# pucgenie/JAADec

Measured on AMD Instinct MI355X. Metric: AAC frames/sec (batched) at 1/2/4/8 MI355X; PCM ±1 LSB vs Java ref, higher is better.
Workload: dtype f32; 1 GPU; C2: 65536 AAC-LC 48 kHz stereo frames (256 streams x 256), ONLY_LONG windows; frames_per_gpu=65536, frames_per_job=65536, streams_per_job=256, parallelism=stream-sharded x1 (no collectives), pcm=int16 big-endian, samples_per_frame=1024, lc_kernel=long-window instantiation

## Files before the change

jaadec_amd/csrc/jaad_lc.hip:

```cpp
#include <hip/hip_runtime.h>

#include <algorithm>

#include "jaad_lc.h"

namespace jaad {

__device__ __forceinline__ int lane_id()
{
    int v;
    asm volatile("v_mbcnt_lo_u32_b32 %0, -1, 0\n\tv_mbcnt_hi_u32_b32 %0, -1, %0" : "=v"(v));
    __builtin_assume(v >= 0 && v < 64);
    return v;
}

__device__ __forceinline__ int lane_pos(int u)
{
    return (u >> 3) | ((int)(__builtin_bitreverse32((uint32_t)u) >> 29) << 3);
}

__device__ __forceinline__ void wave_sync()
{
    __builtin_amdgcn_fence(__ATOMIC_RELEASE, "wavefront");
    __builtin_amdgcn_wave_barrier();
// ... 863 lines not shown
        else if (j == 2) { n = 2 * k + 64; v = re[s]; }
        else { n = 319 - 2 * k; v = re[s]; }
    }
}

__device__ __forceinline__ void ola_short(float* Tb, const LdsTables& T, int u, const FrameCtx& fc,
                                          const float (&re)[8], const float (&im)[8], float (&ov)[16],
                                          float (&out)[16])
{
    const int w = u >> 3, b = u & 7;
    const float* SWc = T.win_short[fc.shape];
    const float* SWr = T.win_short[w == 0 ? fc.shape_prev : fc.shape];
    float nv[16];
#pragma unroll
    for (int phase = 0; phase < 2; phase++) {
#pragma unroll
        for (int s = 0; s < 8; s++) {
#pragma unroll
            for (int j = 0; j < 4; j++) {
                int n;
                float v;
                short_slot(b, s, j, re, im, n, v);
                if ((n < 128) != (phase == 1)) continue;
                if (phase == 0) Tb[128 * w + (n - 128)] = v * SWc[255 - n];
                else Tb[128 * w + n] = v * SWr[n];
            }
        }
        wave_sync();
        const int uu = lane_id();
#pragma unroll
        for (int o = 0; o < 16; o++) {
            const int P = long_pos(uu, o);
            const int mo = (P - 448) >> 7, io = (P - 448) & 127;
            const int mq = (P + 576) >> 7, iq = (P + 576) & 127;
            if (phase == 0) {
                out[o] = (P >= 448 + 128) ? ov[o] + Tb[128 * (mo - 1) + io] : ov[o];
                nv[o] = (mq <= 8) ? Tb[128 * (mq - 1) + iq] : 0.0f;
            } else {
                if (P >= 448) out[o] = out[o] + Tb[128 * mo + io];
                if (mq <= 7) nv[o] = nv[o] + Tb[128 * mq + iq];
            }
        }
        wave_sync();
    }
#pragma unroll
    for (int o = 0; o < 16; o++) ov[o] = nv[o];
}

__device__ __forceinline__ void ola_short2(float* TL, float* TR, const LdsTables& T, int u, const FrameCtx& fL,
                                           const FrameCtx& fR, const float (&reL)[8], const float (&imL)[8],
                                           const float (&reR)[8], const float (&imR)[8], float (&ovL)[16],
                                           float (&ovR)[16], float (&outL)[16], float (&outR)[16])
{
    const int w = u >> 3, b = u & 7;
    const float* SWcL = T.win_short[fL.shape];
    const float* SWrL = T.win_short[w == 0 ? fL.shape_prev : fL.shape];
    const float* SWcR = T.win_short[fR.shape];
    const float* SWrR = T.win_short[w == 0 ? fR.shape_prev : fR.shape];
    float nvL[16], nvR[16];
#pragma unroll
    for (int phase = 0; phase < 2; phase++) {
#pragma unroll
        for (int s = 0; s < 8; s++) {
#pragma unroll
            for (int j = 0; j < 4; j++) {
                int n;
                float vl, vr;
                short_slot(b, s, j, reL, imL, n, vl);
                short_slot(b, s, j, reR, imR, n, vr);
                if ((n < 128) != (phase == 1)) continue;
                if (phase == 0) {
                    TL[128 * w + (n - 128)] = vl * SWcL[255 - n];
                    TR[128 * w + (n - 128)] = vr * SWcR[255 - n];
                } else {
                    TL[128 * w + n] = vl * SWrL[n];
                    TR[128 * w + n] = vr * SWrR[n];
                }
            }
        }
        wave_sync();
        const int uu = lane_id();
#pragma unroll
        for (int o = 0; o < 16; o++) {
            const int P = long_pos(uu, o);
            const int mo = (P - 448) >> 7, io = (P - 448) & 127;
            const int mq = (P + 576) >> 7, iq = (P + 576) & 127;
            if (phase == 0) {
                outL[o] = (P >= 448 + 128) ? ovL[o] + TL[128 * (mo - 1) + io] : ovL[o];
                outR[o] = (P >= 448 + 128) ? ovR[o] + TR[128 * (mo - 1) + io] : ovR[o];
                nvL[o] = (mq <= 8) ? TL[128 * (mq - 1) + iq] : 0.0f;
                nvR[o] = (mq <= 8) ? TR[128 * (mq - 1) + iq] : 0.0f;
            } else {
                if (P >= 448) {
                    outL[o] = outL[o] + TL[128 * mo + io];
                    outR[o] = outR[o] + TR[128 * mo + io];
                }
                if (mq <= 7) {
                    nvL[o] = nvL[o] + TL[128 * mq + iq];
                    nvR[o] = nvR[o] + TR[128 * mq + iq];
                }
            }
        }
        wave_sync();
    }
#pragma unroll
    for (int o = 0; o < 16; o++) {
        ovL[o] = nvL[o];
        ovR[o] = nvR[o];
    }
}

__device__ void tns_spec(float* buf, float* scratch, const LdsTables& T, const GlobalTables& G, int u,
                         const Ics& info, const jaad_tns* tp)
{
    const bool is_short = info.seq == JAAD_EIGHT_SHORT_SEQUENCE;
    const int nswb = is_short ? T.nswb_s : T.nswb_l;
    const int16_t* offs = is_short ? G.swb_s : G.swb_l;
    const int tns_max = is_short ? T.tns_max_s : T.tns_max_l;
    const int nf = tp->n_filters;
    if (u < nf && u < 8) {
        const jaad_tns_filter& F = tp->filt[u];
        int top = nswb, bottom = nswb;
        for (int f = 0; f <= u; f++) {
            const jaad_tns_filter& G = tp->filt[f];
            if (G.window != F.window) continue;
            top = bottom;
            bottom = top - G.length;
            if (bottom < 0) bottom = 0;
        }
        const int order = F.order > 20 ? 20 : F.order;
        float* a = scratch + 24 * u;
        float bb[21];
        const float* tab = G.tns_coef[2 * ((F.flags >> 2) & 1) + ((F.flags >> 1) & 1)];
        a[0] = 1.0f;
        for (int m = 1; m <= order; m++) {
            float tm = -tab[F.coef[m - 1] & 15];
            for (int i = 1; i < m; i++) bb[i] = a[i] + tm * a[m - i];
            for (int i = 1; i < m; i++) a[i] = bb[i];
            a[m] = tm;
        }
        int s = bottom < tns_max ? bottom : tns_max;
        if (s > info.max_sfb) s = info.max_sfb;
        int e = top < tns_max ? top : tns_max;
        if (e > info.max_sfb) e = info.max_sfb;
        int start = offs[s], end = offs[e];
        int size = end - start;
        if (order > 0 && size > 0) {
            int inc = 1;
            if (F.flags & 1) {
                inc = -1;
                start = end - 1;
            }
            const int base = (is_short ? 128 * (F.window & 7) : 0) + start;
            for (int n = 0; n < size; n++) {
                float y = buf[eo_idx(base + n * inc)];
                for (int j = 0; j < order; j++) {
                    float st = (n - 1 - j >= 0) ? buf[eo_idx(base + (n - 1 - j) * inc)] : 0.0f;
                    y -= st * a[j + 1];
                }
                buf[eo_idx(base + n * inc)] = y;
            }
        }
    }
    wave_sync();
}

__device__ __forceinline__ void store_spec(float* buf, int u, const float (&x)[16])
{
#pragma unroll
    for (int h = 0; h < 2; h++) {
        const int p = 8 * u + 512 * h;
        *reinterpret_cast<float4*>(&buf[eo_idx(p)]) = make_float4(x[8 * h], x[8 * h + 2], x[8 * h + 4], x[8 * h + 6]);
        *reinterpret_cast<float4*>(&buf[eo_idx(p + 1)]) =
            make_float4(x[8 * h + 1], x[8 * h + 3], x[8 * h + 5], x[8 * h + 7]);
    }
}
__device__ __forceinline__ void load_spec(const float* buf, int u, float (&x)[16])
{
#pragma unroll
    for (int h = 0; h < 2; h++) {
        const int p = 8 * u + 512 * h;
        float4 e = *reinterpret_cast<const float4*>(&buf[eo_idx(p)]);
        float4 o = *reinterpret_cast<const float4*>(&buf[eo_idx(p + 1)]);
        x[8 * h + 0] = e.x; x[8 * h + 2] = e.y; x[8 * h + 4] = e.z; x[8 * h + 6] = e.w;
        x[8 * h + 1] = o.x; x[8 * h + 3] = o.y; x[8 * h + 5] = o.z; x[8 * h + 7] = o.w;
    }
}

typedef int v4i __attribute__((ext_vector_type(4)));
typedef unsigned v4u __attribute__((ext_vector_type(4)));

__device__ __forceinline__ uint32_t round_pk16(float a, float b)
{
    int ia, ib;
    uint32_t w;
    asm("v_cvt_rpi_i32_f32 %0, %1" : "=v"(ia) : "v"(a));
    asm("v_cvt_rpi_i32_f32 %0, %1" : "=v"(ib) : "v"(b));
    asm("v_cvt_pk_i16_i32 %0, %1, %2" : "=v"(w) : "v"(ia), "v"(ib));
    return w;
}

__device__ __forceinline__ uint32_t round_pk16_lsb1(float a, float b)
{
    f2 x = f2{a, b};
    if constexpr (!kScaledOut) x = x * f2{kPcmUnit, kPcmUnit};
    uint32_t w;
    asm("v_cvt_pknorm_i16_f32 %0, %1, %2" : "=v"(w) : "v"(x.x), "v"(x.y));
    return w;
}

__device__ __forceinline__ void vmem_drain() { __builtin_amdgcn_s_waitcnt(0x0F70); }

__device__ __forceinline__ __amdgpu_buffer_rsrc_t frame_rsrc(void* base, int bytes)
{
    return __builtin_amdgcn_make_buffer_rsrc(base, (short)0, bytes, 0x00020000);
}
__device__ __forceinline__ void store16(v4u v, __amdgpu_buffer_rsrc_t r, int off, bool nt)
{
    if (nt) __builtin_amdgcn_raw_buffer_store_b128(v, r, off, 0, 2);
    else __builtin_amdgcn_raw_buffer_store_b128(v, r, off, 0, 0);
}

constexpr int kRspFloats = kWaveBuf;
template <bool kTns>
struct alignas(16) WaveLds {
    float buf[kWaveBuf];
    float rsp[kRspFloats];
};
template <>
struct alignas(16) WaveLds<true> {
    float buf[kWaveBuf];
    float rsp[kRspFloats];
    float tns[192];
};
#ifndef JAAD_LC_WAVES
#define JAAD_LC_WAVES 12
#endif
template <bool kTns>
constexpr int waves_per_wg()
{
    return kTns ? 8 : JAAD_LC_WAVES;
}

struct alignas(16) BandRec {
    float gl, ms, gr, is;
};
constexpr int kNoBand = 127;
constexpr float kZeroBandGain = -0.0f;

__device__ __forceinline__ int band_short(const LdsTables& T, const Ics& ic, int p)
{
    const int w = p >> 7;
    const int sfb = T.quad2band_s[(p & 127) >> 2];
    const int g = w - __builtin_popcount(ic.grouping & ((1u << w) - 1u));
    return sfb < ic.max_sfb ? g * ic.max_sfb + sfb : kNoBand;
}

__device__ void pns_fill(float* buf, const uint32_t* raw, const LdsTables& T, const GlobalTables& G, int u,
                         const Ics& info)
{
    if (u == 0) {
        const uint8_t* sfr = reinterpret_cast<const uint8_t*>(raw);
        const uint8_t* cbr = sfr + 128;
        const bool is_short = info.seq == JAAD_EIGHT_SHORT_SEQUENCE;
        const int16_t* offs = is_short ? G.swb_s : G.swb_l;
        int glen[8], ng = 1;
        glen[0] = 1;
        if (is_short)
            for (int i = 0; i < 7; i++) {
                if (info.grouping & (1u << i)) glen[ng - 1]++;
                else glen[ng++] = 1;
            }
        uint32_t rs = info.pns;
        const int maxSFB = info.max_sfb;
        for (int g = 0, idx = 0, groupOff = 0; g < ng; g++) {
            for (int sfb = 0; sfb < maxSFB; sfb++, idx++) {
                if (cbr[idx] != JAAD_NOISE_HCB) continue;
                int off = groupOff + offs[sfb];
                const int width = offs[sfb + 1] - offs[sfb];
                const float sfv = -T.sf_gain[sfr[idx]];
                for (int w = 0; w < glen[g]; w++, off += 128) {
                    float energy = 0.0f;
                    for (int k = 0; k < width; k++) {
                        rs = 1664525u * rs + 1013904223u;
                        const float v = (float)(int32_t)rs;
                        buf[eo_idx(off + k)] = v;
                        energy += v * v;
                    }
                    const float scale = (float)((double)sfv / sqrt((double)energy));
                    for (int k = 0; k < width; k++) buf[eo_idx(off + k)] *= scale;
                }
            }
            groupOff += glen[g] << 7;
        }
    }
    wave_sync();
}

struct Prefetch {
    v4i q[2][2];
    uint32_t sf2[2], cb2[2];
    uint32_t side;
};

__device__ __forceinline__ void prefetch(const KernelArgs& A, int f, bool stereo, int u, Prefetch& pf, int skip = 0)
{
    const int nch = stereo ? 2 : 1;
#pragma unroll
    for (int c = 0; c < 2; c++) {
        if (c == 1 && !stereo) break;
        const size_t cf = (size_t)f * A.cf_stride + c;
        const v4i* q = reinterpret_cast<const v4i*>(A.q + cf * 1024);
        pf.q[c][0] = __builtin_nontemporal_load(q + u);
        pf.q[c][1] = __builtin_nontemporal_load(q + 64 + u);
        pf.sf2[c] = reinterpret_cast<const uint16_t*>(A.sf + cf * 128)[u];
        pf.cb2[c] = reinterpret_cast<const uint16_t*>(A.cb + cf * 128)[u];
    }
    const uint32_t* side = u < 8 ? reinterpret_cast<const uint32_t*>(A.ics + (size_t)f * A.cf_stride) + (u < 4 * nch ? u : 0)
                                 : (A.ms_used ? reinterpret_cast<const uint32_t*>(A.ms_used + (size_t)f * 2 * A.ms_stride) + (u & 3)
                                              : reinterpret_cast<const uint32_t*>(A.ics));
    if (A.skips && u >= 62) side = A.skips + 2 * skip + (u == 62);
    pf.side = *side;
}

__device__ __forceinline__ void iq_channel(const LdsTables& T, const float* iq_global, const v4i (&q)[2],
                                           const float (&g)[4], float (&x)[16])
{
    float v[16];
    typedef unsigned short us2 __attribute__((ext_vector_type(2)));
    static_assert(kIqHead == 1024, "escape mask assumes a 2048-entry head");
    uint32_t t[8];
#pragma unroll
    for (int d = 0; d < 8; d++) {
        const uint32_t w = reinterpret_cast<const uint32_t*>(&q[d >> 2])[d & 3];
        t[d] = __builtin_bit_cast(uint32_t, __builtin_bit_cast(us2, w) + (us2){kIqHead, kIqHead});
    }
    const bool esc = ((t[0] | t[1] | t[2] | t[3] | t[4] | t[5] | t[6] | t[7]) & 0xF800F800u) != 0u;
#pragma unroll
    for (int e = 0; e < 16; e++) {
        const uint32_t idx = (e & 1) ? (t[e >> 1] >> 16) : (t[e >> 1] & 0xFFFFu);
        v[e] = T.iq_signed[idx];
    }
    __builtin_amdgcn_sched_group_barrier(0x0002, 8, 0);
#pragma unroll
    for (int e = 0; e < 16; e++) {
        __builtin_amdgcn_sched_group_barrier(0x0002, 1, 0);
        __builtin_amdgcn_sched_group_barrier(0x0100, 1, 0);
    }
    __builtin_amdgcn_sched_group_barrier(0x0002, 64, 0);
#pragma unroll
    for (int e = 0; e < 16; e++) {
        const float gn = g[e >> 2];
        x[e] = v[e] * gn;
    }
    if (__builtin_expect(__ballot(esc) != 0, 0)) {
#pragma unroll
        for (int e = 0; e < 16; e++) {
            const int qq = reinterpret_cast<const int16_t*>(&q[e >> 3])[e & 7];
            const int qc = qq < -kIqHead ? -kIqHead : (qq > kIqHead - 1 ? kIqHead - 1 : qq);
            const int aq = qq < 0 ? -qq : qq;
            const float gn = g[e >> 2];
            const float m = iq_global[aq > 8190 ? 8190 : aq] * gn;
            const bool big = (qq > kIqHead - 1 || qq < -kIqHead) && gn != 0.0f;
            x[e] = big ? (qq > 0 ? m : -m) : T.iq_signed[qc + kIqHead] * gn;
        }
    }
}

struct IqPending {
    float v[16];
    bool esc;
};
__device__ __forceinline__ void iq_issue(const LdsTables& T, const v4i (&q)[2], IqPending& P)
{
    typedef unsigned short us2 __attribute__((ext_vector_type(2)));
    uint32_t t[8];
#pragma unroll
    for (int d = 0; d < 8; d++) {
        const uint32_t w = reinterpret_cast<const uint32_t*>(&q[d >> 2])[d & 3];
        t[d] = __builtin_bit_cast(uint32_t, __builtin_bit_cast(us2, w) + (us2){kIqHead, kIqHead});
    }
    P.esc = ((t[0] | t[1] | t[2] | t[3] | t[4] | t[5] | t[6] | t[7]) & 0xF800F800u) != 0u;
#pragma unroll
    for (int e = 0; e < 16; e++) {
        const uint32_t idx = (e & 1) ? (t[e >> 1] >> 16) : (t[e >> 1] & 0xFFFFu);
        P.v[e] = T.iq_signed[idx];
    }
}
__device__ __forceinline__ void iq_finish(const LdsTables& T, const float* iq_global, const v4i (&q)[2],
                                          const IqPending& P, const float (&g)[4], float (&x)[16])
{
#pragma unroll
    for (int e = 0; e < 16; e++) x[e] = P.v[e] * g[e >> 2];
    if (__builtin_expect(__ballot(P.esc) != 0, 0)) {
#pragma unroll
        for (int e = 0; e < 16; e++) {
            const int qq = reinterpret_cast<const int16_t*>(&q[e >> 3])[e & 7];
            const int qc = qq < -kIqHead ? -kIqHead : (qq > kIqHead - 1 ? kIqHead - 1 : qq);
            const int aq = qq < 0 ? -qq : qq;
            const float gn = g[e >> 2];
            const float m = iq_global[aq > 8190 ? 8190 : aq] * gn;
            const bool big = (qq > kIqHead - 1 || qq < -kIqHead) && gn != 0.0f;
            x[e] = big ? (qq > 0 ? m : -m) : T.iq_signed[qc + kIqHead] * gn;
        }
    }
}

__device__ __forceinline__ void couple_after_tns(const KernelArgs& A, float* buf, int f, int ch, int u)
{
    const uint32_t t0 = A.cce_off[f], t1 = A.cce_off[f + 1];
    bool any = false;
    float x[16];
    for (uint32_t t = t0; t < t1; t++) {
        const uint32_t meta = A.cce_meta[t];
        if (!(meta >> 24) || (int)((meta >> 16) & 0xFF) - (int)A.ch0 != ch) continue;
        if (!any) load_spec(buf, u, x);
        any = true;
        const float4* sp = reinterpret_cast<const float4*>(A.cce_spec + (size_t)t * 1024);
#pragma unroll
        for (int h = 0; h < 2; h++) {
            const float4 a = sp[(512 * h + 8 * u) / 4], c = sp[(512 * h + 8 * u) / 4 + 1];
            const float v[8] = {a.x, a.y, a.z, a.w, c.x, c.y, c.z, c.w};
#pragma unroll
            for (int i = 0; i < 8; i++) x[8 * h + i] += v[i];
        }
    }
    if (any) {
        store_spec(buf, u, x);
        wave_sync();
    }
}

template <bool kTnsSpec, bool kCoupleAfter = false, bool F = false>
__device__ __forceinline__ void synth_channel(const KernelArgs& A, const LdsTables& T, WaveLds<kTnsSpec>& W, float* buf,
                                              const Ics& ic, size_t cf, float (&ov)[16], float (&out)[16], int f = 0,
                                              int ch = 0)
{
    const int u = lane_id();
    if constexpr (kTnsSpec)
        if (A.tns_mode == JAAD_TNS_SPEC && (ic.flags & JAAD_ICS_TNS) && A.tns) tns_spec(buf, W.tns, T, *A.gtab, u, ic, A.tns + cf);
    if constexpr (kCoupleAfter) couple_after_tns(A, buf, f, ch, u);
    const FrameCtx fc{ic.seq, ic.shape, ic.shape_prev};
    if (fc.seq == JAAD_EIGHT_SHORT_SEQUENCE) {
        float re[8], im[8];
        imdct_short_pk<F>(buf, T, u, re, im);
        ola_short(buf, T, u, fc, re, im, ov, out);
    } else {
        float* const bufs[1] = {buf};
        f2 cx[1][8];
        imdct_long_pk<1, F>(bufs, T, u, cx);
        ola_long_pk<F>(T, fc, cx[0], ov, out);
    }
    wave_sync();
}

#ifdef JAAD_STAMPS
#define STAMP(k)                                                  \
    do {                                                          \
        uint64_t t_;                                              \
        asm volatile("s_memtime %0\n\ts_waitcnt lgkmcnt(0)" : "=s"(t_)::"memory"); \
        st_acc[k] += (uint32_t)(t_ - st_prev);                    \
        st_prev = t_;                                             \
    } while (0)
#elif defined(JAAD_MARKS)
#define STAMP(k) asm volatile(";PHASE " #k)
#else
#define STAMP(k) \
    do {         \
    } while (0)
#endif

#ifdef JAAD_BOUNDS
#define JAAD_BOUND(ci, f, cond, what, a, b)                                                                 \
    do {                                                                                                   \
        if (!(cond)) {                                                                                     \
            if (lane_id() == 0)                                                                            \
                printf("JAAD_BOUNDS lc_decode_kernel: chunk %u frame %d: %s %u vs %u\n", (unsigned)(ci), (int)(f), \
                       what, (unsigned)(a), (unsigned)(b));                                                \
            return;                                                                                        \
        }                                                                                                  \
    } while (0)
#else
#define JAAD_BOUND(ci, f, cond, what, a, b) \
    do {                                    \
    } while (0)
#endif

template <int kMode, int kOut, bool kStereo>
__global__ __launch_bounds__(64 * waves_per_wg<kMode == 1 || kMode == 3>()) void lc_decode_kernel(KernelArgs A)
{
    constexpr bool kTnsSpec = kMode == 1 || kMode == 3;
    [[maybe_unused]] constexpr bool kCouple = kMode == 2 || kMode == 3;
    constexpr bool kFast = kMode == 4 || kMode == 6;
    [[maybe_unused]] constexpr bool kShortPair = kMode == 5 || kMode == 6;
    constexpr int kW = waves_per_wg<kTnsSpec>();
    constexpr int kThreads = 64 * kW;
    struct Lds {
        LdsTables T;
        WaveLds<kTnsSpec> W[kW];
        uint32_t rem[kW];
    };
    __shared__ Lds S;
    LdsTables& T = S.T;

    {
        const uint4* src = reinterpret_cast<const uint4*>(A.tables);
        uint4* dst = reinterpret_cast<uint4*>(&T);
        for (int i = threadIdx.x; i < (int)(sizeof(LdsTables) / 16); i += kThreads) dst[i] = src[i];
        if (threadIdx.x < kW) S.rem[threadIdx.x] = 0u;
    }
    __syncthreads();
#ifdef JAAD_WAVETIME
    const uint64_t wt0 = __builtin_amdgcn_s_memrealtime();
    uint32_t wt_frames = 0;
#endif

    constexpr bool big_endian = !(kOut & JAAD_PCM_LITTLE_ENDIAN);
    constexpr bool planar = kOut == (int)kOutPlanarF32;
    constexpr bool out_f32 = (kOut & JAAD_PCM_FLOAT32) != 0 && !planar;
    [[maybe_unused]] constexpr bool out_i16 = !planar && !out_f32;
    const int wave = __builtin_amdgcn_readfirstlane(threadIdx.x >> 6);
    constexpr bool stereo = kStereo;
    constexpr int nch = stereo ? 2 : 1;
    WaveLds<kTnsSpec>& W = S.W[wave];
    BandRec* rec = reinterpret_cast<BandRec*>(W.buf);

    const int nswb_l = __builtin_amdgcn_readfirstlane(T.nswb_l), nswb_s = __builtin_amdgcn_readfirstlane(T.nswb_s);
    uint32_t q2b_long = 0;
    {
        const int u = lane_id();
#pragma unroll
        for (int qd = 0; qd < 4; qd++) {
            const uint32_t b = T.quad2band_l[(512 * (qd >> 1) + 8 * u + 4 * (qd & 1)) >> 2];
            q2b_long |= (b > kNoBand ? kNoBand : b) << (8 * qd);
        }
    }

#ifdef JAAD_STAMPS
    uint32_t st_acc[16] = {};
    uint64_t st_prev;
    asm volatile("s_memtime %0\n\ts_waitcnt lgkmcnt(0)" : "=s"(st_prev)::"memory");
#endif
    for (uint32_t ci = blockIdx.x * kW + wave; ci < A.n_chunks; ci += gridDim.x * kW) {
        const ChunkDesc cd = A.chunks[ci];
        const int nfr = cd.info & 0xffff;
        const bool prefix = (cd.info & kChunkPrefix) != 0;
        const int my_n = nfr + (prefix ? 1 : 0);
        const int f_first = (int)cd.frame0;
        JAAD_BOUND(ci, -1, cd.slot < A.n_slots, "chunk slot", cd.slot, A.n_slots);
        JAAD_BOUND(ci, f_first, my_n == 0 || (cd.frame0 >= A.frame_lo && cd.frame0 + (uint32_t)my_n <= A.frame_hi),
                   "chunk frames", cd.frame0 + (uint32_t)my_n, A.frame_hi);
        JAAD_BOUND(ci, f_first, !A.skips || cd.skip < A.n_skip_pairs, "chunk skip entry", cd.skip, A.n_skip_pairs);
        if (cd.slot >= A.n_slots || (my_n && (cd.frame0 < A.frame_lo || cd.frame0 >= A.frame_hi))) continue;

        float ovL[16], ovR[16];
        {
            const int u = lane_id();
            if (cd.info & kChunkLoadState) {
                const float* st = A.state_in + (size_t)cd.slot * 2048;
#pragma unroll
                for (int o = 0; o < 16; o++) {
                    ovL[o] = st[long_pos(u, o)];
                    ovR[o] = st[1024 + long_pos(u, o)];
                    if constexpr (kFast && kScaledOut) {
                        ovL[o] *= kPcmUnit;
                        ovR[o] *= kPcmUnit;
                    }
                }
            } else {
#pragma unroll
                for (int o = 0; o < 16; o++) ovL[o] = ovR[o] = 0.0f;
            }
        }
        int skip = (int)cd.skip;
        int fr_next = f_first;
        Prefetch pf;
        if (my_n > 0) prefetch(A, fr_next, stereo, lane_id(), pf, skip);
        vmem_drain();

        for (int it = 0; it < my_n; it++) {
#if !defined(JAAD_ABL_NOPRIO)
#ifndef JAAD_PRIO_EVERY
#define JAAD_PRIO_EVERY 1
#endif
            if ((it % JAAD_PRIO_EVERY) == 0) {
                const uint32_t rem = (uint32_t)(my_n - it);
                int p = 0;
                if constexpr (kFast) {
                    __hip_atomic_store(&S.rem[wave], rem, __ATOMIC_RELAXED, __HIP_MEMORY_SCOPE_WORKGROUP);
                    uint32_t mates[kW / 4 - 1];
#pragma unroll
                    for (int m = 1; m < kW / 4; m++)
                        mates[m - 1] = __hip_atomic_load(&S.rem[(wave + 4 * m) % kW], __ATOMIC_RELAXED, __HIP_MEMORY_SCOPE_WORKGROUP);
                    static_assert(kW <= 16, "the key keeps the wave in 4 bits");
                    const uint32_t key = (rem << 4) | (uint32_t)wave;
#pragma unroll
                    for (int m = 1; m < kW / 4; m++) {
                        const uint32_t mate = (uint32_t)((wave + 4 * m) % kW);
                        p += key > ((__builtin_amdgcn_readfirstlane(mates[m - 1]) << 4) | mate) ? 1 : 0;
                    }
                } else {
                    volatile uint32_t* R = S.rem;
                    R[wave] = rem;
#pragma unroll
                    for (int m = 1; m < kW / 4; m++) {
                        const int mate = (wave + 4 * m) % kW;
                        const uint32_t r = __builtin_amdgcn_readfirstlane(R[mate]);
                        p += (rem > r || (rem == r && wave > mate)) ? 1 : 0;
                    }
                }
                if (p >= 2) __builtin_amdgcn_s_setprio(3);
                else if (p == 1) __builtin_amdgcn_s_setprio(2);
                else __builtin_amdgcn_s_setprio(1);
            }
#endif
            STAMP(5);
#ifdef JAAD_WAVETIME
            wt_frames++;
#endif
            const int u = lane_id();
            const bool emit = it >= (prefix ? 1 : 0);
            const int f = fr_next;
            const size_t cf0 = (size_t)f * A.cf_stride;
            const Prefetch cur = pf;
            fr_next = f + 1;
            if (A.skips && fr_next == __builtin_amdgcn_readlane(cur.side, 63)) {
                fr_next += __builtin_amdgcn_readlane(cur.side, 62);
                skip++;
            }
            JAAD_BOUND(ci, f, (uint32_t)f >= A.frame_lo && (uint32_t)f < A.frame_hi, "frame rows / pcm", f, A.frame_hi);
            JAAD_BOUND(ci, f, it + 1 >= my_n || ((uint32_t)fr_next >= A.frame_lo && (uint32_t)fr_next < A.frame_hi),
                       "prefetched frame", fr_next, A.frame_hi);
            JAAD_BOUND(ci, f, !A.skips || (uint32_t)skip < A.n_skip_pairs, "skip entry", skip, A.n_skip_pairs);
            if constexpr (kCouple) {
                JAAD_BOUND(ci, f, A.cce_off[f] <= A.cce_off[f + 1] && A.cce_off[f + 1] <= A.n_cce_terms, "coupling terms",
                           A.cce_off[f + 1], A.n_cce_terms);
            }

#if defined(JAAD_NO_IQ_EARLY)
            constexpr bool kIqEarly = false;
#else
            constexpr bool kIqEarly = kFast;
#endif
            [[maybe_unused]] IqPending iqL, iqR;
            if constexpr (kIqEarly) {
                iq_issue(T, cur.q[0], iqL);
                if (stereo) iq_issue(T, cur.q[1], iqR);
            }
            const Ics iL = ics_from_lanes(cur.side, 0, nswb_l, nswb_s);
            STAMP(6);
            const Ics iR = stereo ? ics_from_lanes(cur.side, 4, nswb_l, nswb_s) : iL;
            const bool ms_on = stereo && (iL.flags & JAAD_ICS_COMMON_WINDOW) && (iL.flags & JAAD_ICS_MS_PRESENT);
            const bool is_on = stereo && (iR.flags & JAAD_ICS_HAS_IS);
            const bool same_bands = !stereo || (iL.seq == iR.seq && iL.max_sfb == iR.max_sfb && iL.grouping == iR.grouping);
            uint64_t m0 = 0, m1 = 0;
            if (ms_on && A.ms_used) {
                m0 = (uint64_t)(uint32_t)__builtin_amdgcn_readlane(cur.side, 8) |
                     ((uint64_t)(uint32_t)__builtin_amdgcn_readlane(cur.side, 9) << 32);
                m1 = (uint64_t)(uint32_t)__builtin_amdgcn_readlane(cur.side, 10) |
                     ((uint64_t)(uint32_t)__builtin_amdgcn_readlane(cur.side, 11) << 32);
            }

            STAMP(0);
            {
                const uint32_t sfL2 = cur.sf2[0], cbL2 = cur.cb2[0];
                const uint32_t sfR2 = stereo ? cur.sf2[1] : 0u, cbR2 = stereo ? cur.cb2[1] : 0u;
                const uint64_t mw = u < 32 ? m0 : m1;
                const uint32_t msb = (uint32_t)(mw >> ((2 * u) & 63)) & 3u;
                BandRec br[2];
#pragma unroll
                for (int e = 0; e < 2; e++) {
                    const int b = 2 * u + e;
                    const uint32_t sfL = (sfL2 >> (8 * e)) & 255u, cbL = (cbL2 >> (8 * e)) & 255u;
                    const uint32_t sfR = (sfR2 >> (8 * e)) & 255u, cbR = (cbR2 >> (8 * e)) & 255u;
                    const bool inL = b < iL.nbands, inR = b < iR.nbands;
                    const bool msbit = (msb >> e) & 1u;
                    const float gvL = T.sf_gain[sfL];
                    br[e].gl = (inL && cbL != JAAD_ZERO_HCB && cbL < JAAD_NOISE_HCB) ? gvL : kZeroBandGain;
                    br[e].ms = (ms_on && inL && msbit && cbL < JAAD_NOISE_HCB && cbR < JAAD_NOISE_HCB) ? 1.0f : 0.0f;
                    float gr = 0.0f, is = 0.0f;
                    if (stereo) {
                        const float gvR = T.sf_gain[sfR];
                        gr = (inR && cbR != JAAD_ZERO_HCB && cbR < JAAD_NOISE_HCB) ? gvR : kZeroBandGain;
                        if (is_on && inR && (cbR == JAAD_INTENSITY_HCB || cbR == JAAD_INTENSITY_HCB2)) {
                            float cs = cbR == JAAD_INTENSITY_HCB ? 1.0f : -1.0f;
                            if ((iL.flags & JAAD_ICS_MS_PRESENT) && msbit) cs = -cs;
                            is = cs * gvR;
                        }
                    }
                    br[e].gr = gr;
                    br[e].is = is;
                }
                wave_sync();
                reinterpret_cast<float4*>(rec)[2 * u] = make_float4(br[0].gl, br[0].ms, br[0].gr, br[0].is);
                reinterpret_cast<float4*>(rec)[2 * u + 1] = make_float4(br[1].gl, br[1].ms, br[1].gr, br[1].is);
            }
            wave_sync();

            STAMP(1);
            float gL[4], gR[4], msq[4], isq[4];
            uint32_t q2b = q2b_long;
            asm volatile("" : "+v"(q2b));
            if (iL.seq != JAAD_EIGHT_SHORT_SEQUENCE && same_bands) {
#pragma unroll
                for (int qd = 0; qd < 4; qd++) {
                    const float4 r = reinterpret_cast<const float4*>(rec)[(q2b >> (8 * qd)) & 255u];
                    gL[qd] = r.x;
                    msq[qd] = r.y;
                    gR[qd] = r.z;
                    isq[qd] = r.w;
                }
            } else {
#pragma unroll
                for (int qd = 0; qd < 4; qd++) {
                    const int p = 512 * (qd >> 1) + 8 * u + 4 * (qd & 1);
                    const int bl = iL.seq == JAAD_EIGHT_SHORT_SEQUENCE ? band_short(T, iL, p) : (int)((q2b >> (8 * qd)) & 255u);
                    const float4 r = reinterpret_cast<const float4*>(rec)[bl];
                    gL[qd] = r.x;
                    msq[qd] = r.y;
                    if (same_bands) {
                        gR[qd] = r.z;
                        isq[qd] = r.w;
                    } else {
                        const int br = iR.seq == JAAD_EIGHT_SHORT_SEQUENCE ? band_short(T, iR, p) : (int)((q2b >> (8 * qd)) & 255u);
                        const float2 rr = reinterpret_cast<const float2*>(rec)[2 * br + 1];
                        gR[qd] = rr.x;
                        isq[qd] = rr.y;
                    }
                }
            }
            float xL[16], xR[16];
            STAMP(14);
            if constexpr (kIqEarly) {
                iq_finish(T, A.iq_table, cur.q[0], iqL, gL, xL);
                STAMP(13);
                if (stereo) iq_finish(T, A.iq_table, cur.q[1], iqR, gR, xR);
            } else {
                iq_channel(T, A.iq_table, cur.q[0], gL, xL);
                STAMP(13);
                if (stereo) iq_channel(T, A.iq_table, cur.q[1], gR, xR);
            }
            STAMP(12);
#ifdef JAAD_ABL_NOPREF
            if (it == 0)
#endif
            prefetch(A, it + 1 < my_n ? fr_next : f, stereo, u, pf, skip);

            if ((iL.flags | (stereo ? iR.flags : 0)) & JAAD_ICS_HAS_PNS) {
                uint32_t* rcopy = reinterpret_cast<uint32_t*>(W.rsp);
                wave_sync();
                {
                    uint16_t* r16 = reinterpret_cast<uint16_t*>(rcopy);
                    r16[u] = (uint16_t)cur.sf2[0];
                    r16[64 + u] = (uint16_t)cur.cb2[0];
                    if (stereo) {
                        r16[128 + u] = (uint16_t)cur.sf2[1];
                        r16[192 + u] = (uint16_t)cur.cb2[1];
                    }
                }
                if (iL.flags & JAAD_ICS_HAS_PNS) {
                    wave_sync();
                    store_spec(W.buf, u, xL);
                    wave_sync();
                    pns_fill(W.buf, rcopy, T, *A.gtab, u, iL);
                    load_spec(W.buf, u, xL);
                }
                if (stereo && (iR.flags & JAAD_ICS_HAS_PNS)) {
                    wave_sync();
                    store_spec(W.buf, u, xR);
                    wave_sync();
                    pns_fill(W.buf, rcopy + 64, T, *A.gtab, u, iR);
                    load_spec(W.buf, u, xR);
                }
            }
            STAMP(2);
            if (ms_on) {
#pragma unroll
                for (int qd = 0; qd < 4; qd++) {
                    if (msq[qd] != 0.0f) {
#pragma unroll
                        for (int i = 0; i < 4; i++) {
                            const int e = 8 * (qd >> 1) + 4 * (qd & 1) + i;
                            const float l = xL[e], r = xR[e];
                            xL[e] = l + r;
                            xR[e] = l - r;
                        }
                    }
                }
            }
            if (is_on) {
#pragma unroll
                for (int qd = 0; qd < 4; qd++) {
                    if (isq[qd] != 0.0f) {
#pragma unroll
                        for (int i = 0; i < 4; i++) {
                            const int e = 8 * (qd >> 1) + 4 * (qd & 1) + i;
                            xR[e] = xL[e] * isq[qd];
                        }
                    }
                }
            }

            if constexpr (kCouple) {
                const uint32_t t0 = A.cce_off[f], t1 = A.cce_off[f + 1];
                for (uint32_t t = t0; t < t1; t++) {
                    if (kMode == 3 && (A.cce_meta[t] >> 24)) break;
                    const int ch = (int)((A.cce_meta[t] >> 16) & 0xFF) - (int)A.ch0;
                    if (ch < 0 || ch >= nch) continue;
                    const float4* sp = reinterpret_cast<const float4*>(A.cce_spec + (size_t)t * 1024);
                    float v[16];
#pragma unroll
                    for (int h = 0; h < 2; h++) {
                        const float4 a = sp[(512 * h + 8 * u) / 4], c = sp[(512 * h + 8 * u) / 4 + 1];
                        v[8 * h + 0] = a.x;
                        v[8 * h + 1] = a.y;
                        v[8 * h + 2] = a.z;
                        v[8 * h + 3] = a.w;
                        v[8 * h + 4] = c.x;
                        v[8 * h + 5] = c.y;
                        v[8 * h + 6] = c.z;
                        v[8 * h + 7] = c.w;
                    }
                    if (ch == 0) {
#pragma unroll
                        for (int e = 0; e < 16; e++) xL[e] += v[e];
                    } else {
                        if constexpr (stereo) {
#pragma unroll
                            for (int e = 0; e < 16; e++) xR[e] += v[e];
                        }
                    }
                }
            }

            STAMP(3);
            wave_sync();
            store_spec(W.buf, u, xL);
            if (stereo) store_spec(W.rsp, u, xR);
            wave_sync();
            STAMP(4);
            float outL[16], outR[16];
            if (stereo && iL.seq != JAAD_EIGHT_SHORT_SEQUENCE && iR.seq != JAAD_EIGHT_SHORT_SEQUENCE) {
                if constexpr (kTnsSpec) {
                    if (A.tns_mode == JAAD_TNS_SPEC && A.tns) {
                        if (iL.flags & JAAD_ICS_TNS) tns_spec(W.buf, W.tns, T, *A.gtab, u, iL, A.tns + cf0);
                        if (iR.flags & JAAD_ICS_TNS) tns_spec(W.rsp, W.tns, T, *A.gtab, u, iR, A.tns + cf0 + 1);
                    }
                }
                if constexpr (kMode == 3) {
                    couple_after_tns(A, W.buf, f, 0, u);
                    couple_after_tns(A, W.rsp, f, 1, u);
                }
                float* const bufs[2] = {W.buf, W.rsp};
                f2 cx[2][8];
                imdct_long_pk<2, kFast>(bufs, T, lane_id(), cx);
                ola_long_pk<kFast>(T, FrameCtx{iL.seq, iL.shape, iL.shape_prev}, cx[0], ovL, outL);
                ola_long_pk<kFast>(T, FrameCtx{iR.seq, iR.shape, iR.shape_prev}, cx[1], ovR, outR);
                wave_sync();
            } else if (kShortPair && stereo && iL.seq == JAAD_EIGHT_SHORT_SEQUENCE && iR.seq == JAAD_EIGHT_SHORT_SEQUENCE) {
                float reL[8], imL[8], reR[8], imR[8];
                imdct_short_pk2<kFast>(W.buf, W.rsp, T, lane_id(), reL, imL, reR, imR);
                ola_short2(W.buf, W.rsp, T, lane_id(), FrameCtx{iL.seq, iL.shape, iL.shape_prev},
                           FrameCtx{iR.seq, iR.shape, iR.shape_prev}, reL, imL, reR, imR, ovL, ovR, outL, outR);
                wave_sync();
            } else {
                synth_channel<kTnsSpec, kMode == 3, kFast>(A, T, W, W.buf, iL, cf0, ovL, outL, f, 0);
                if (stereo) synth_channel<kTnsSpec, kMode == 3, kFast>(A, T, W, W.rsp, iR, cf0 + 1, ovR, outR, f, 1);
            }
            STAMP(8);
            vmem_drain();
            STAMP(9);
            {
                const int u2 = lane_id();
                const int drop = emit ? 0 : 4096;
                if constexpr (planar) {
#pragma unroll
                    for (int o = 0; o < 16; o++) {
                        W.buf[long_pos(u2, o)] = kFast && kScaledOut ? outL[o] * kPcmScale : outL[o];
                        if (stereo) W.rsp[long_pos(u2, o)] = kFast && kScaledOut ? outR[o] * kPcmScale : outR[o];
                    }
                    wave_sync();
#pragma unroll
                    for (int c = 0; c < nch; c++) {
                        const __amdgpu_buffer_rsrc_t dst = frame_rsrc(reinterpret_cast<float*>(A.pcm) + (cf0 + c) * 1024, 4096);
                        const float* srcb = c ? W.rsp : W.buf;
#pragma unroll
                        for (int jj = 0; jj < 4; jj++)
                            store16(*reinterpret_cast<const v4u*>(srcb + 4 * u2 + 256 * jj), dst, 16 * u2 + 1024 * jj + drop, false);
                    }
                    wave_sync();
                } else if constexpr (out_f32) {
                    typedef unsigned v2u __attribute__((ext_vector_type(2)));
                    const __amdgpu_buffer_rsrc_t dst = frame_rsrc(reinterpret_cast<uint8_t*>(A.pcm) + (size_t)f * 8192, 8192);
                    const int drop8 = emit ? 0 : 8192;
#pragma unroll
                    for (int o = 0; o < 16; o++) {
                        const float sl = kFast && kScaledOut ? outL[o] * kPcmScale : outL[o];
                        const float sr = stereo ? (kFast && kScaledOut ? outR[o] * kPcmScale : outR[o]) : sl;
                        const v2u w = {__float_as_uint(sl), __float_as_uint(sr)};
                        __builtin_amdgcn_raw_buffer_store_b64(w, dst, 8 * long_pos(u2, o) + drop8, 0, 0);
                    }
                } else {
                    const uint32_t sel0 = big_endian ? 0x04050001u : 0x05040100u;
                    const uint32_t sel1 = big_endian ? 0x06070203u : 0x07060302u;
                    uint32_t* stage = reinterpret_cast<uint32_t*>(W.buf);
#ifdef JAAD_ABL_NOPCM
                    if (f < 0)
#endif
#pragma unroll
                    for (int m = 0; m < 8; m++) {
                        uint32_t pl, pr;
#if defined(JAAD_NO_PKNORM)
                        constexpr bool kPkNorm = false;
#else
                        constexpr bool kPkNorm = kFast;
#endif
                        if constexpr (kPkNorm) {
                            pl = round_pk16_lsb1(outL[2 * m], outL[2 * m + 1]);
                            pr = stereo ? round_pk16_lsb1(outR[2 * m], outR[2 * m + 1]) : pl;
                        } else if constexpr (kFast && kScaledOut) {
                            pl = round_pk16(outL[2 * m] * kPcmScale, outL[2 * m + 1] * kPcmScale);
                            pr = stereo ? round_pk16(outR[2 * m] * kPcmScale, outR[2 * m + 1] * kPcmScale) : pl;
                        } else {
                            pl = round_pk16(outL[2 * m], outL[2 * m + 1]);
                            pr = stereo ? round_pk16(outR[2 * m], outR[2 * m + 1]) : pl;
                        }
                        stage[long_pos(u2, 2 * m)] = __builtin_amdgcn_perm(pr, pl, sel0);
                        stage[long_pos(u2, 2 * m + 1)] = __builtin_amdgcn_perm(pr, pl, sel1);
                    }
                    wave_sync();
                    const __amdgpu_buffer_rsrc_t dst = frame_rsrc(reinterpret_cast<uint8_t*>(A.pcm) + (size_t)f * 4096, 4096);
#pragma unroll
                    for (int jj = 0; jj < 4; jj++)
                        store16(*reinterpret_cast<const v4u*>(stage + 4 * u2 + 256 * jj), dst, 16 * u2 + 1024 * jj + drop, true);
                    wave_sync();
                }
            }
            STAMP(10);
        }
        STAMP(11);
        if constexpr (kFast) __hip_atomic_store(&S.rem[wave], 0u, __ATOMIC_RELAXED, __HIP_MEMORY_SCOPE_WORKGROUP);
        else reinterpret_cast<volatile uint32_t*>(S.rem)[wave] = 0u;
        if (cd.info & kChunkStoreState) {
            const int u = lane_id();
            float* st = A.state_out + (size_t)cd.slot * 2048;
            constexpr float sc = kFast && kScaledOut ? kPcmScale : 1.0f;
#pragma unroll
            for (int o = 0; o < 16; o++) {
                st[long_pos(u, o)] = kFast && kScaledOut ? ovL[o] * sc : ovL[o];
                if (stereo) st[1024 + long_pos(u, o)] = kFast && kScaledOut ? ovR[o] * sc : ovR[o];
            }
        }
    }
#ifdef JAAD_WAVETIME
    {
        const uint64_t wt1 = __builtin_amdgcn_s_memrealtime();
        if (A.dbg && lane_id() == 0) {
            uint64_t* o = reinterpret_cast<uint64_t*>(A.dbg) + (size_t)(blockIdx.x * kW + wave) * 4;
            o[0] = wt0;
            o[1] = wt1;
            o[2] = (uint64_t)__builtin_amdgcn_s_getreg((20 << 0) | (0 << 6) | (3 << 11));
            o[3] = (uint64_t)wt_frames;
        }
    }
#endif
#ifdef JAAD_STAMPS
    if (A.dbg && lane_id() == 0) {
        uint32_t* o = reinterpret_cast<uint32_t*>(A.dbg) + (size_t)(blockIdx.x * kW + wave) * 16;
        for (int k = 0; k < 16; k++) o[k] = st_acc[k];
    }
#endif
}

template <int kMode, bool kStereo>
static void launch_lc_mode(const KernelArgs& a, hipStream_t stream)
{
    constexpr int W = waves_per_wg<kMode == 1 || kMode == 3>();
#define JAAD_LAUNCH(O) \
    hipLaunchKernelGGL((lc_decode_kernel<kMode, O, kStereo>), dim3((a.n_chunks + W - 1) / W), dim3(64 * W), 0, stream, a)
    const int o = (a.out_mode == kOutPlanarF32) ? 4 : (a.out_mode & JAAD_PCM_FLOAT32) ? 2 : (a.out_mode & JAAD_PCM_LITTLE_ENDIAN) ? 1 : 0;
    if (o == 4) JAAD_LAUNCH(kOutPlanarF32);
    else if (o == 2) JAAD_LAUNCH(JAAD_PCM_FLOAT32);
    else if (o == 1) JAAD_LAUNCH(JAAD_PCM_LITTLE_ENDIAN);
    else JAAD_LAUNCH(JAAD_PCM_BIG_ENDIAN);
#undef JAAD_LAUNCH
}

hipError_t launch_lc_fast(const KernelArgs& a, hipStream_t stream);

#ifndef JAAD_LC_FAST_TU
template <bool kStereo>
static hipError_t launch_lc_ch(const KernelArgs& a, hipStream_t stream, bool tns_spec)
{
    if (a.cce_off && tns_spec) launch_lc_mode<3, kStereo>(a, stream);
    else if (a.cce_off) launch_lc_mode<2, kStereo>(a, stream);
    else if (tns_spec) launch_lc_mode<1, kStereo>(a, stream);
    else if (a.precision == JAAD_PRECISION_LSB1) return launch_lc_fast(a, stream);
    else {
        if constexpr (kStereo)
            if (a.short_pair) {
                launch_lc_mode<5, kStereo>(a, stream);
                return hipGetLastError();
            }
        launch_lc_mode<0, kStereo>(a, stream);
    }
    return hipGetLastError();
}

namespace {
__device__ __forceinline__ bool frame_skipped(const uint32_t* __restrict__ skips, uint32_t n, uint32_t f)
{
    uint32_t lo = 0, hi = n;
    while (lo < hi) {
        const uint32_t m = (lo + hi) >> 1;
        if (skips[2 * m] <= f) lo = m + 1;
        else hi = m;
    }
    return lo > 0 && f - skips[2 * (lo - 1)] < skips[2 * (lo - 1) + 1];
}

__global__ __launch_bounds__(256) void pack_kernel(const float* __restrict__ planar, void* __restrict__ pcm,
                                                   uint32_t n_frames, int n_ch, uint32_t flags,
                                                   const uint32_t* __restrict__ skips, uint32_t n_skips)
{
    const size_t i = (size_t)blockIdx.x * 256 + threadIdx.x;
    if (i >= (size_t)n_frames * 1024) return;
    const size_t f = i >> 10, n = i & 1023;
    if (n_skips && frame_skipped(skips, n_skips, (uint32_t)f)) return;
    const float* src = planar + f * (size_t)n_ch * 1024 + n;
    if (flags & JAAD_PCM_FLOAT32) {
        float* o = reinterpret_cast<float*>(pcm) + i * n_ch;
        for (int c = 0; c < n_ch; c++) o[c] = src[(size_t)c * 1024];
        return;
    }
    uint16_t* o = reinterpret_cast<uint16_t*>(pcm) + i * n_ch;
    for (int c = 0; c < n_ch; c++) {
        uint32_t s16 = round_pk16(src[(size_t)c * 1024], 0.0f) & 0xFFFFu;
        if (!(flags & JAAD_PCM_LITTLE_ENDIAN)) s16 = ((s16 & 0xFF) << 8) | (s16 >> 8);
        o[c] = (uint16_t)s16;
    }
}
}

namespace {
__global__ __launch_bounds__(256) void check_q_kernel(const v4i* __restrict__ q, size_t n16, int* __restrict__ flag)
{
    int bad = 0;
    for (size_t i = (size_t)blockIdx.x * 256 + threadIdx.x; i < n16; i += (size_t)gridDim.x * 256) {
        const v4i w = __builtin_nontemporal_load(q + i);
#pragma unroll
        for (int k = 0; k < 4; k++) {
            const int lo = (int)(int16_t)(w[k] & 0xFFFF), hi = w[k] >> 16;
            bad |= (lo > 8190) | (lo < -8190) | (hi > 8190) | (hi < -8190);
        }
    }
    if (bad) *flag = 1;
}
}

namespace {
__global__ __launch_bounds__(64) void cce_term_kernel(CceArgs A)
{
    __shared__ float buf[kWaveBuf];
    __shared__ uint32_t raw[64];
    const uint32_t t = blockIdx.x;
    if (t >= A.n_terms) return;
    const int u = lane_id();
    const LdsTables& T = *A.tables;
    const uint32_t rec = A.meta[t] & 0xFFFFu;
    const jaad_ics_info ic = A.ics[rec];
    Ics info;
    info.seq = ic.window_sequence & 3;
    info.shape = ic.window_shape & 1;
    info.shape_prev = ic.window_shape_prev & 1;
    const int lim = info.seq == JAAD_EIGHT_SHORT_SEQUENCE ? T.nswb_s : T.nswb_l;
    info.max_sfb = min((int)ic.max_sfb, lim);
    info.grouping = ic.grouping;
    info.flags = ic.flags;
    info.pns = ic.pns_state;
    const int groups = info.seq == JAAD_EIGHT_SHORT_SEQUENCE ? 8 - __builtin_popcount(info.grouping & 0x7f) : 1;
    info.nbands = groups * info.max_sfb;
    raw[u] = reinterpret_cast<const uint32_t*>(u < 32 ? A.sf + (size_t)rec * 128 : A.cb + (size_t)rec * 128)[u & 31];
    wave_sync();
    const uint8_t* sfr = reinterpret_cast<const uint8_t*>(raw);
    const uint8_t* cbr = sfr + 128;
    const int16_t* q = A.q + (size_t)rec * 1024;
    const float* gain = A.gain + (size_t)t * 120;
    float x[16], g[16];
    bool touched[16];
#pragma unroll
    for (int e = 0; e < 16; e++) {
        const int p = 512 * (e >> 3) + 8 * u + (e & 7);
        int band = kNoBand;
        if (info.seq == JAAD_EIGHT_SHORT_SEQUENCE) {
            band = band_short(T, info, p & ~3);
        } else {
            const int b = T.quad2band_l[p >> 2];
            band = b < info.max_sfb ? b : kNoBand;
        }
        x[e] = 0.0f;
        g[e] = 0.0f;
        touched[e] = false;
        if (band == kNoBand) continue;
        const int c = cbr[band];
        touched[e] = c != JAAD_ZERO_HCB;
        g[e] = gain[band];
        if (c != JAAD_ZERO_HCB && c < JAAD_NOISE_HCB) {
            const int v = q[p];
            const int a = min(v < 0 ? -v : v, 8190);
            const float iq = v > 0 ? A.iq_table[a] : -A.iq_table[a];
            x[e] = iq * T.sf_gain[sfr[band]];
        }
    }
    if (info.flags & JAAD_ICS_HAS_PNS) {
        wave_sync();
        store_spec(buf, u, x);
        wave_sync();
        pns_fill(buf, raw, T, *A.gtab, u, info);
        load_spec(buf, u, x);
    }
    float* out = A.spec + (size_t)t * 1024;
#pragma unroll
    for (int e = 0; e < 16; e++) out[512 * (e >> 3) + 8 * u + (e & 7)] = touched[e] ? g[e] * x[e] : -0.0f;
}
}

hipError_t launch_cce_terms(const CceArgs& a, hipStream_t stream)
{
    if (!a.n_terms) return hipSuccess;
    hipLaunchKernelGGL(cce_term_kernel, dim3(a.n_terms), dim3(64), 0, stream, a);
    return hipGetLastError();
}

hipError_t launch_check_q(const int16_t* q, size_t n, int* flag, hipStream_t stream)
{
    const size_t n16 = n / 8;
    if (!n16) return hipSuccess;
    const unsigned blocks = (unsigned)std::min<size_t>((n16 + 255) / 256, 2048);
    hipLaunchKernelGGL(check_q_kernel, dim3(blocks), dim3(256), 0, stream, reinterpret_cast<const v4i*>(q), n16, flag);
    return hipGetLastError();
}

namespace {
template <typename W>
__global__ __launch_bounds__(256) void mc_interleave_kernel(McInterleave m, W* __restrict__ out, size_t n,
                                                            uint32_t samples, const uint32_t* __restrict__ skips,
                                                            uint32_t n_skips)
{
    const size_t i = (size_t)blockIdx.x * 256 + threadIdx.x;
    if (i >= n) return;
    if (n_skips && frame_skipped(skips, n_skips, (uint32_t)(i / samples))) return;
    W* o = out + i * m.n_out;
    for (int c = 0; c < m.n_out; c++) o[c] = static_cast<const W*>(m.src[c])[2 * i + m.chan[c]];
}
}

hipError_t launch_mc_interleave(const McInterleave& m, void* pcm, uint32_t n_frames, uint32_t samples, int bps,
                                hipStream_t stream, const uint32_t* skips, uint32_t n_skips)
{
    const size_t n = (size_t)n_frames * samples;
    if (!n) return hipSuccess;
    if (m.n_out < 1 || m.n_out > 16) return hipErrorInvalidValue;
    const dim3 grid((unsigned)((n + 255) / 256));
    if (bps == 4)
        hipLaunchKernelGGL(mc_interleave_kernel<uint32_t>, grid, dim3(256), 0, stream, m, static_cast<uint32_t*>(pcm), n,
                           samples, skips, n_skips);
    else
        hipLaunchKernelGGL(mc_interleave_kernel<uint16_t>, grid, dim3(256), 0, stream, m, static_cast<uint16_t*>(pcm), n,
                           samples, skips, n_skips);
    return hipGetLastError();
}

hipError_t launch_pack(const float* planar, void* pcm, uint32_t n_frames, int n_ch, uint32_t flags, hipStream_t stream,
                       const uint32_t* skips, uint32_t n_skips)
{
    const size_t n = (size_t)n_frames * 1024;
    if (!n) return hipSuccess;
    hipLaunchKernelGGL(pack_kernel, dim3((unsigned)((n + 255) / 256)), dim3(256), 0, stream, planar, pcm, n_frames, n_ch,
                       flags, skips, n_skips);
    return hipGetLastError();
}

hipError_t launch_lc(const KernelArgs& a, hipStream_t stream, bool tns_spec)
{
    return a.nch == 2 ? launch_lc_ch<true>(a, stream, tns_spec) : launch_lc_ch<false>(a, stream, tns_spec);
}

int lc_resident_waves_per_cu(bool tns_spec)
{
    int blocks = 0;
    hipError_t e = tns_spec ? hipOccupancyMaxActiveBlocksPerMultiprocessor(&blocks, lc_decode_kernel<1, JAAD_PCM_BIG_ENDIAN, true>,
                                                                            64 * waves_per_wg<true>(), 0)
                            : hipOccupancyMaxActiveBlocksPerMultiprocessor(&blocks, lc_decode_kernel<0, JAAD_PCM_BIG_ENDIAN, true>,
                                                                            64 * waves_per_wg<false>(), 0);
    if (e != hipSuccess) return 0;
    return blocks * (tns_spec ? waves_per_wg<true>() : waves_per_wg<false>());
}
#else
hipError_t launch_lc_fast(const KernelArgs& a, hipStream_t stream)
{
    if (a.nch == 2) {
        if (a.short_pair) launch_lc_mode<6, true>(a, stream);
        else launch_lc_mode<4, true>(a, stream);
    } else {
        launch_lc_mode<4, false>(a, stream);
    }
    return hipGetLastError();
}
#endif

}
```

Before: 412.4 million frames/s.

## Relayout side loads for DPP MS bits, scalarize priority, unroll frame loop by two

In fast modes the prefetch now loads the M/S mask words with one dword per 16-lane row. Each lane then pulls its MS bits with a single DPP row broadcast instead of four readlanes plus 64-bit shifts, and the skip lanes move to 16/17. The wave-priority comparison is rewritten as SALU s_cmp/s_addc inline asm, with monotonic setprio calls. When JAAD_LC_FAST_TU is defined, the frame loop body becomes an always-inline lambda called twice per iteration, so the compiler can interleave consecutive frames. These changes cut scalar/VALU overhead per frame at the cost of code size and register pressure from the unroll.

```diff
diff --git a/jaadec_amd/csrc/jaad_lc.hip b/jaadec_amd/csrc/jaad_lc.hip
--- a/jaadec_amd/csrc/jaad_lc.hip
+++ b/jaadec_amd/csrc/jaad_lc.hip
@@ -1189,7 +1189,18 @@
     uint32_t sf2[2], cb2[2];
     uint32_t side;
 };
-
+#if defined(JAAD_MS_READLANE)
+constexpr bool kSideByRow = false;
+#else
+constexpr bool kSideByRow = true;
+#endif
+template <bool F>
+constexpr int skip_lane()
+{
+    return F && kSideByRow ? 17 : 63;
+}
+
+template <bool F>
 __device__ __forceinline__ void prefetch(const KernelArgs& A, int f, bool stereo, int u, Prefetch& pf, int skip = 0)
 {
     const int nch = stereo ? 2 : 1;
@@ -1202,6 +1213,15 @@
         pf.q[c][1] = __builtin_nontemporal_load(q + 64 + u);
         pf.sf2[c] = reinterpret_cast<const uint16_t*>(A.sf + cf * 128)[u];
         pf.cb2[c] = reinterpret_cast<const uint16_t*>(A.cb + cf * 128)[u];
+    }
+    if constexpr (F && kSideByRow) {
+        const uint32_t* side = u < 8 ? reinterpret_cast<const uint32_t*>(A.ics + (size_t)f * A.cf_stride) + (u < 4 * nch ? u : 0)
+                                     : (A.ms_used ? reinterpret_cast<const uint32_t*>(A.ms_used + (size_t)f * 2 * A.ms_stride) + (u >> 4)
+                                                  : reinterpret_cast<const uint32_t*>(A.ics));
+        constexpr int ks = skip_lane<F>();
+        if (A.skips && (u | 1) == ks) side = A.skips + 2 * skip + (u == ks - 1);
+        pf.side = *side;
+        return;
     }
     const uint32_t* side = u < 8 ? reinterpret_cast<const uint32_t*>(A.ics + (size_t)f * A.cf_stride) + (u < 4 * nch ? u : 0)
                                  : (A.ms_used ? reinterpret_cast<const uint32_t*>(A.ms_used + (size_t)f * 2 * A.ms_stride) + (u & 3)
@@ -1357,6 +1377,7 @@
     } while (0)
 #endif
 
+#define JAAD_BOUND_RETURN return
 #ifdef JAAD_BOUNDS
 #define JAAD_BOUND(ci, f, cond, what, a, b)                                                                 \
     do {                                                                                                   \
@@ -1364,7 +1385,7 @@
             if (lane_id() == 0)                                                                            \
                 printf("JAAD_BOUNDS lc_decode_kernel: chunk %u frame %d: %s %u vs %u\n", (unsigned)(ci), (int)(f), \
                        what, (unsigned)(a), (unsigned)(b));                                                \
-            return;                                                                                        \
+            JAAD_BOUND_RETURN;                                                                             \
         }                                                                                                  \
     } while (0)
 #else
@@ -1462,10 +1483,17 @@
         int skip = (int)cd.skip;
         int fr_next = f_first;
         Prefetch pf;
-        if (my_n > 0) prefetch(A, fr_next, stereo, lane_id(), pf, skip);
+        if (my_n > 0) prefetch<kFast>(A, fr_next, stereo, lane_id(), pf, skip);
         vmem_drain();
 
+#if defined(JAAD_LC_FAST_TU) && !defined(JAAD_NO_UNROLL2)
+#define JAAD_FRAME_LAMBDA
+#undef JAAD_BOUND_RETURN
+#define JAAD_BOUND_RETURN return false
+        const auto frame = [&](const int it) __attribute__((always_inline)) -> bool {
+#else
         for (int it = 0; it < my_n; it++) {
+#endif
 #if !defined(JAAD_ABL_NOPRIO)
 #ifndef JAAD_PRIO_EVERY
 #define JAAD_PRIO_EVERY 1
@@ -1484,7 +1512,13 @@
 #pragma unroll
                     for (int m = 1; m < kW / 4; m++) {
                         const uint32_t mate = (uint32_t)((wave + 4 * m) % kW);
-                        p += key > ((__builtin_amdgcn_readfirstlane(mates[m - 1]) << 4) | mate) ? 1 : 0;
+                        const uint32_t mkey = (__builtin_amdgcn_readfirstlane(mates[m - 1]) << 4) | mate;
+#if defined(JAAD_PRIO_VALU)
+                        p += key > mkey ? 1 : 0;
+#else
+                        if (m == 1) asm("s_cmp_gt_u32 %1, %2\n\ts_cselect_b32 %0, 1, 0" : "=s"(p) : "s"(key), "s"(mkey) : "scc");
+                        else asm("s_cmp_gt_u32 %1, %2\n\ts_addc_u32 %0, %0, 0" : "+s"(p) : "s"(key), "s"(mkey) : "scc");
+#endif
                     }
                 } else {
                     volatile uint32_t* R = S.rem;
@@ -1496,6 +1530,13 @@
                         p += (rem > r || (rem == r && wave > mate)) ? 1 : 0;
                     }
                 }
+#if !defined(JAAD_PRIO_VALU)
+                if constexpr (kFast) {
+                    __builtin_amdgcn_s_setprio(1);
+                    if (p >= 1) __builtin_amdgcn_s_setprio(2);
+                    if (p >= 2) __builtin_amdgcn_s_setprio(3);
+                } else
+#endif
                 if (p >= 2) __builtin_amdgcn_s_setprio(3);
                 else if (p == 1) __builtin_amdgcn_s_setprio(2);
                 else __builtin_amdgcn_s_setprio(1);
@@ -1511,8 +1552,8 @@
             const size_t cf0 = (size_t)f * A.cf_stride;
             const Prefetch cur = pf;
             fr_next = f + 1;
-            if (A.skips && fr_next == __builtin_amdgcn_readlane(cur.side, 63)) {
-                fr_next += __builtin_amdgcn_readlane(cur.side, 62);
+            if (A.skips && fr_next == __builtin_amdgcn_readlane(cur.side, skip_lane<kFast>())) {
+                fr_next += __builtin_amdgcn_readlane(cur.side, skip_lane<kFast>() - 1);
                 skip++;
             }
             JAAD_BOUND(ci, f, (uint32_t)f >= A.frame_lo && (uint32_t)f < A.frame_hi, "frame rows / pcm", f, A.frame_hi);
@@ -1540,8 +1581,10 @@
             const bool ms_on = stereo && (iL.flags & JAAD_ICS_COMMON_WINDOW) && (iL.flags & JAAD_ICS_MS_PRESENT);
             const bool is_on = stereo && (iR.flags & JAAD_ICS_HAS_IS);
             const bool same_bands = !stereo || (iL.seq == iR.seq && iL.max_sfb == iR.max_sfb && iL.grouping == iR.grouping);
+            constexpr bool kMsByRow = kFast && kSideByRow;
+            const bool ms_bits = ms_on && A.ms_used;
             uint64_t m0 = 0, m1 = 0;
-            if (ms_on && A.ms_used) {
+            if (!kMsByRow && ms_bits) {
                 m0 = (uint64_t)(uint32_t)__builtin_amdgcn_readlane(cur.side, 8) |
                      ((uint64_t)(uint32_t)__builtin_amdgcn_readlane(cur.side, 9) << 32);
                 m1 = (uint64_t)(uint32_t)__builtin_amdgcn_readlane(cur.side, 10) |
@@ -1552,8 +1595,14 @@
             {
                 const uint32_t sfL2 = cur.sf2[0], cbL2 = cur.cb2[0];
                 const uint32_t sfR2 = stereo ? cur.sf2[1] : 0u, cbR2 = stereo ? cur.cb2[1] : 0u;
-                const uint64_t mw = u < 32 ? m0 : m1;
-                const uint32_t msb = (uint32_t)(mw >> ((2 * u) & 63)) & 3u;
+                uint32_t msb;
+                if constexpr (kMsByRow) {
+                    const uint32_t mw = (uint32_t)__builtin_amdgcn_update_dpp((int)cur.side, (int)cur.side, 0x128, 0xf, 0x3, false);
+                    msb = (mw >> ((2 * u) & 31)) & 3u;
+                } else {
+                    const uint64_t mw = u < 32 ? m0 : m1;
+                    msb = (uint32_t)(mw >> ((2 * u) & 63)) & 3u;
+                }
                 BandRec br[2];
 #pragma unroll
                 for (int e = 0; e < 2; e++) {
@@ -1564,14 +1613,14 @@
                     const bool msbit = (msb >> e) & 1u;
                     const float gvL = T.sf_gain[sfL];
                     br[e].gl = (inL && cbL != JAAD_ZERO_HCB && cbL < JAAD_NOISE_HCB) ? gvL : kZeroBandGain;
-                    br[e].ms = (ms_on && inL && msbit && cbL < JAAD_NOISE_HCB && cbR < JAAD_NOISE_HCB) ? 1.0f : 0.0f;
+                    br[e].ms = ((kMsByRow ? ms_bits : ms_on) && inL && msbit && cbL < JAAD_NOISE_HCB && cbR < JAAD_NOISE_HCB) ? 1.0f : 0.0f;
                     float gr = 0.0f, is = 0.0f;
                     if (stereo) {
                         const float gvR = T.sf_gain[sfR];
                         gr = (inR && cbR != JAAD_ZERO_HCB && cbR < JAAD_NOISE_HCB) ? gvR : kZeroBandGain;
                         if (is_on && inR && (cbR == JAAD_INTENSITY_HCB || cbR == JAAD_INTENSITY_HCB2)) {
                             float cs = cbR == JAAD_INTENSITY_HCB ? 1.0f : -1.0f;
-                            if ((iL.flags & JAAD_ICS_MS_PRESENT) && msbit) cs = -cs;
+                            if ((kMsByRow ? ms_bits : (iL.flags & JAAD_ICS_MS_PRESENT) != 0) && msbit) cs = -cs;
                             is = cs * gvR;
                         }
                     }
@@ -1631,7 +1680,7 @@
 #ifdef JAAD_ABL_NOPREF
             if (it == 0)
 #endif
-            prefetch(A, it + 1 < my_n ? fr_next : f, stereo, u, pf, skip);
+            prefetch<kFast>(A, it + 1 < my_n ? fr_next : f, stereo, u, pf, skip);
 
             if ((iL.flags | (stereo ? iR.flags : 0)) & JAAD_ICS_HAS_PNS) {
                 uint32_t* rcopy = reinterpret_cast<uint32_t*>(W.rsp);
@@ -1824,7 +1873,20 @@
                 }
             }
             STAMP(10);
-        }
+#ifdef JAAD_FRAME_LAMBDA
+            return true;
+        };
+#undef JAAD_BOUND_RETURN
+#define JAAD_BOUND_RETURN return
+        static_assert(kFast, "only the +-1 LSB modes are built with the unrolled frame loop");
+        for (int it = 0; it < my_n; it += 2) {
+            if (!frame(it)) return;
+            if (it + 1 >= my_n) break;
+            if (!frame(it + 1)) return;
+        }
+#else
+        }
+#endif
         STAMP(11);
         if constexpr (kFast) __hip_atomic_store(&S.rem[wave], 0u, __ATOMIC_RELAXED, __HIP_MEMORY_SCOPE_WORKGROUP);
         else reinterpret_cast<volatile uint32_t*>(S.rem)[wave] = 0u;
```

After: 419.2 million frames/s, median of 6. +1.6%, better.
